# Project-Arda/bgls

Measured on AMD Instinct MI355X. Metric: aggregate-verify signer-pairs/sec, higher is better.
Workload: dtype u32; 1 GPU; altbn128 VerifyAggregateSignature, one 1048576-signer batch, keys+msgs resident in HBM; curve=altbn128, signers=1048576, signers_per_gpu=1048576, in_flight=8

## Files before the change

### __graft_entry__.py

```python
import os
import subprocess
import sys

ROOT = os.path.dirname(os.path.abspath(__file__))
HIPCC = os.environ.get("HIPCC", "/opt/rocm/bin/hipcc")


def _run(cmd, timeout=1800):
    print("+", " ".join(cmd), flush=True)
    subprocess.run(cmd, check=True, cwd=ROOT, timeout=timeout)


def build(force=False):
    csrc = os.path.join(ROOT, "bgls_amd", "csrc")
    jobs = str(min(8, os.cpu_count() or 1))
    _run(["make", "-s", "-j", jobs, "-C", csrc, "HIPCC=" + HIPCC] + (["-B"] if force else []))
    _run(["make", "-s", "-j", jobs, "-C", csrc, "HIPCC=" + HIPCC, "LEGACY=1"] + (["-B"] if force else []))
    omk = os.path.join(ROOT, "oracle", "c", "Makefile")
    if os.path.exists(omk):
        _run(["make", "-s", "-C", os.path.join(ROOT, "oracle", "c")])
    bh_path = os.path.join(ROOT, "tests", "harness", "build_harness.py")
    if os.path.exists(bh_path):
        import importlib.util
        spec = importlib.util.spec_from_file_location("build_harness", bh_path)
        bh = importlib.util.module_from_spec(spec)
        spec.loader.exec_module(bh)
        print("+ host harness (test-only, five parts in parallel)", flush=True)
        bh.build(force=force)
    dh_path = os.path.join(ROOT, "tests", "harness", "build_device_harness.py")
    if os.path.exists(dh_path):
        import importlib.util
        spec = importlib.util.spec_from_file_location("build_device_harness", dh_path)
        dh = importlib.util.module_from_spec(spec)
        spec.loader.exec_module(dh)
        print("+ device harness (test-only, gfx950)", flush=True)
        dh.build(force=force)
    sys.path.insert(0, ROOT)
    import bgls_amd
    from bgls_amd import _lib
    _lib.load()


def smoke():
    sys.path.insert(0, ROOT)
    import ctypes, random
    from bgls_amd import Altbn128, Bls12, bgls, _lib
    from oracle import coracle
    rc = _lib.load().bgls_init(0)
    if rc != 0:
        raise RuntimeError("bgls_init failed: %d %s" % (rc, _lib.last_error()))
    for curve in (Altbn128, Bls12):
        cid = curve.id
        n = 4
        sks = [0x1234567 + 977 * i for i in range(n)]
        msgs = [bytes([i]) * (17 + i) for i in range(n)]
        keys = [curve.GetG2().Mul(sk) for sk in sks]
        sigs = [bgls.Sign(curve, sk, m) for sk, m in zip(sks, msgs)]
        agg = bgls.AggregateSignatures(sigs)
        g2 = curve.GetG2().raw
        okeys = [coracle.scale_point(cid, 2, g2, sk) for sk in sks]
        osigs = [coracle.scale_point(cid, 1, coracle.hash_to_g1(cid, m), sk) for sk, m in zip(sks, msgs)]
        oagg = coracle.aggregate_points(cid, 1, b"".join(osigs), n)
        assert [k.raw for k in keys] == okeys, "public keys differ from oracle"
        assert agg.raw == oagg, "aggregate signature differs from oracle"
        got = bgls.VerifyAggregateSignature(curve, agg, keys, msgs)
        want = coracle.verify_aggregate(cid, oagg, b"".join(okeys), msgs, False, threads=4)
        assert got is True and want == 1, (curve.Name(), got, want)
        bad = bgls.VerifyAggregateSignature(curve, agg, keys, msgs[:-1] + [b"tampered"])
        assert bad is False, "tampered message accepted"
        lib, fp = _lib.load(), curve.fp_bytes
        rnd = random.Random(7)
        n = 150
        sks = [rnd.randrange(1, curve.GetG1Order()) for _ in range(n)]
        kb = (ctypes.c_uint8 * (32 * n)).from_buffer_copy(b"".join(s.to_bytes(32, "big") for s in sks))
        kbuf = (ctypes.c_uint8 * (n * 4 * fp))()
        assert lib.bgls_scale_generator(cid, 2, kb, n, kbuf) == 0
        ms = [rnd.randbytes(32) for _ in range(n)]
        blob = (ctypes.c_uint8 * (32 * n)).from_buffer_copy(b"".join(ms))
        off = (ctypes.c_uint64 * (n + 1))(*range(0, 32 * (n + 1), 32))
        sg = (ctypes.c_uint8 * (n * 2 * fp))()
        assert lib.bgls_sign_batch(cid, kb, blob, off, n, sg) == 0
        ag = (ctypes.c_uint8 * (2 * fp))()
        assert lib.bgls_aggregate_points(cid, 1, sg, n, ag) == 0
        assert lib.bgls_verify_aggregate(cid, ag, kbuf, blob, off, n, 0) == 1
        assert coracle.verify_aggregate(cid, bytes(ag), bytes(kbuf), ms, False, threads=8) == 1, "oracle disagrees on the 150-signer instance"
        blob[32 * 77 + 5] ^= 4
        assert lib.bgls_verify_aggregate(cid, ag, kbuf, blob, off, n, 0) == 0, "tampered 150-signer instance accepted"
        print("smoke ok:", curve.Name())


if __name__ == "__main__":
    build()
    if len(sys.argv) > 1 and sys.argv[1] == "smoke":
        smoke()
```

### bgls_amd/csrc/miller_x.hpp

```cpp
#pragma once
#include <type_traits>
#include "dev_common.hpp"
#include "coop.hpp"
#include "rx_pair.hpp"

namespace bgls {

template <class C>
struct MxForm { typedef C type; };
#ifndef MX_BN_W28
template <>
struct MxForm<BN254> { typedef BN254W type; };
#endif

template <class C, int NP = 60>
struct MX {
  static_assert(NP == 60 || NP == 64, "pairings per block");
  static constexpr int NL = C::RX_NL;
  static constexpr bool PACKED = (C::RX_NL % 4) != 0 && C::CURVE_ID == 1;
  static constexpr int HS = PACKED ? NL : ((NL + 3) & ~3);
  static constexpr int ES = 2 * HS;
  static constexpr int NLINES = NP == 64 ? 7 : 6;
  static constexpr int FOLD_UNROLL = (!rx_lazy<C> && NLINES % 3 == 0) ? 3 : 1;
  static constexpr int KS = PACKED ? 2 * ES : ES;
  static constexpr int WS = PACKED ? 368 : 176;
  static constexpr int GROUP_DW = PACKED ? (NP == 64 ? 940 : 844) : (NP == 64 ? 828 : 764);
  static constexpr int THREADS = 192;
  static __device__ __forceinline__ int acc_off(int k, int wrap) { return k * KS + wrap * WS; }
  static __device__ __forceinline__ int line_off(int e) {
    if constexpr (PACKED) return e < 12 ? 28 + 56 * e + (e >= 6 ? 32 : 0) : (e == 12 ? 336 : 704 + 28 * (e - 13));
    else return 320 + ES * e;
  }
  static_assert(!PACKED || (ES == 28 && 704 + 28 * (3 * NLINES - 13) <= GROUP_DW), "BLS12-381 line slots");
  static_assert(PACKED || 320 + ES * 3 * NLINES <= GROUP_DW, "alt-bn128 line slots");
  static constexpr int PQ = 10 * GROUP_DW;
#ifndef MX_P_LDS_LIMIT
#define MX_P_LDS_LIMIT 40960
#endif
  static constexpr bool P_IN_LDS = (10 * GROUP_DW + NP * 2 * HS) * 4 <= MX_P_LDS_LIMIT;
  static constexpr int SEQ_DW = 10 * GROUP_DW + (P_IN_LDS ? NP * 2 * HS : 0);
#ifdef MX_EXP_FLAGS
  static constexpr int BLOCK_BYTES = (SEQ_DW + 16) * 4;
#else
  static constexpr int BLOCK_BYTES = (10 * GROUP_DW + (P_IN_LDS ? NP * 2 * HS : 0)) * 4;
#endif
  static constexpr int NPARK_Q = C::CURVE_ID == 0 ? 6 : 2;
  static constexpr int NPARK = NPARK_Q + (P_IN_LDS ? 0 : 2);
  static constexpr int PS = (NL + 3) & ~3;
  static constexpr size_t park_bytes(size_t nblocks) { return nblocks * 128 * NPARK * PS * 4; }
};

__device__ __forceinline__ uint4 mx_ld16(int dw) {
  extern __shared__ u32 lds[];
  typedef u32 v4u __attribute__((ext_vector_type(4)));
  const v4u v = *reinterpret_cast<const v4u*>(__builtin_assume_aligned(lds + dw, 16));
  return make_uint4(v.x, v.y, v.z, v.w);
}
template <class C, bool PACKED>
__device__ __forceinline__ Ux<C> mx_ld_half(int off, bool second) {
  constexpr int N = C::RX_NL;
  Ux<C> r;
  if constexpr (!PACKED) {
    (void)second;
#pragma unroll
    for (int k = 0; k < (N + 3) / 4; ++k) {
      const uint4 v = mx_ld16(off + 4 * k);
      r.v[4 * k] = v.x;
      if (4 * k + 1 < N) r.v[4 * k + 1] = v.y;
      if (4 * k + 2 < N) r.v[4 * k + 2] = v.z;
      if (4 * k + 3 < N) r.v[4 * k + 3] = v.w;
    }
  } else {
    static_assert(!PACKED || N % 4 == 2, "packed halves: NL = 2 mod 4");
    if (!second) {
#pragma unroll
      for (int k = 0; k < (N + 2) / 4; ++k) {
        const uint4 v = mx_ld16(off + 4 * k);
        r.v[4 * k] = v.x; r.v[4 * k + 1] = v.y;
        if (4 * k + 2 < N) { r.v[4 * k + 2] = v.z; r.v[4 * k + 3] = v.w; }
      }
    } else {
      const uint4 v0 = mx_ld16(off - 2);
      r.v[0] = v0.z; r.v[1] = v0.w;
#pragma unroll
      for (int k = 1; k < (N + 2) / 4; ++k) {
        const uint4 v = mx_ld16(off - 2 + 4 * k);
        r.v[4 * k - 2] = v.x; r.v[4 * k - 1] = v.y; r.v[4 * k] = v.z; r.v[4 * k + 1] = v.w;
      }
    }
  }
  return r;
}
template <class C, bool PACKED>
__device__ __forceinline__ void mx_st_half(int off, bool second, const Ux<C>& a) {
  extern __shared__ u32 lds[];
  constexpr int N = C::RX_NL;
  if (!PACKED || !second) {
    uint4* p = reinterpret_cast<uint4*>(lds + off);
#pragma unroll
    for (int k = 0; k < N / 4; ++k) p[k] = make_uint4(a.v[4 * k], a.v[4 * k + 1], a.v[4 * k + 2], a.v[4 * k + 3]);
    if constexpr (N % 4 == 2) *reinterpret_cast<uint2*>(lds + off + (N & ~3)) = make_uint2(a.v[N - 2], a.v[N - 1]);
    if constexpr (N % 4 == 1) lds[off + N - 1] = a.v[N - 1];
    static_assert(N % 4 != 3, "tail store");
  } else {
    *reinterpret_cast<uint2*>(lds + off) = make_uint2(a.v[0], a.v[1]);
    uint4* p = reinterpret_cast<uint4*>(lds + off + 2);
#pragma unroll
    for (int k = 0; k < N / 4; ++k) p[k] = make_uint4(a.v[4 * k + 2], a.v[4 * k + 3], a.v[4 * k + 4], a.v[4 * k + 5]);
  }
}

template <class C, class K, bool XI3 = false>
__device__ __forceinline__ void mxk_publish(int gb, int j, const Ux2<C>& v, bool live) {
  if (live) {
    mx_st_half<C, K::PACKED>(gb + K::acc_off(j, 0), false, v.c0);
    mx_st_half<C, K::PACKED>(gb + K::acc_off(j, 0) + K::HS, true, v.c1);
    const Ux2<C> x = ux_mulxi<C>(v);
    if (!XI3 || j >= 3) {
      mx_st_half<C, K::PACKED>(gb + K::acc_off(j, 1), false, x.c0);
      mx_st_half<C, K::PACKED>(gb + K::acc_off(j, 1) + K::HS, true, x.c1);
    }
  }
  wave_sync();
}
template <class C, int NP>
__device__ __forceinline__ void mx_publish(int gb, int j, const Ux2<C>& v, bool live) { mxk_publish<C, MX<C, NP>>(gb, j, v, live); }
template <class C, int NP>
__device__ __forceinline__ Ux2<C> mx_fold(int gb, int m, int j) {
  typedef MX<C, NP> K;
  auto sh = [](int t) { return C::TWIST_D ? t + (t == 2 ? 1 : 0) : t + (t >= 1 ? 1 : 0); };
#ifdef MX_EXP_Q
  if constexpr (C::RX_NL <= 10)
    return ux_dot_k2q<C, 3>(
      [&](int t, int h) { return mx_ld_half<C, K::PACKED>(gb + K::line_off(3 * m + t) + h * K::HS, h != 0); },
      [&](int t, int h) {
        int k = j - sh(t);
        const int wrap = k < 0 ? 1 : 0;
        k += 6 * wrap;
        return mx_ld_half<C, K::PACKED>(gb + K::acc_off(k, wrap) + h * K::HS, h != 0);
      });
  else
#endif
  return ux_dot_k2p<C, 3, (C::RX_NL <= 10)>(
      [&](int t, int h) { return mx_ld_half<C, K::PACKED>(gb + K::line_off(3 * m + t) + h * K::HS, h != 0); },
      [&](int t, int h) {
        int k = j - sh(t);
        const int wrap = k < 0 ? 1 : 0;
        k += 6 * wrap;
        return mx_ld_half<C, K::PACKED>(gb + K::acc_off(k, wrap) + h * K::HS, h != 0);
      });
}
template <class C, class K>
__device__ __forceinline__ Ux2<C> mxk_sqr(int gb, int j) {
  const unsigned row = COOP_SQ_TAB[j];
  return ux_sqr_dot<C>(
      [&](int t) {
        const unsigned e = (row >> (8 * t)) & 0xFFu;
        return (e & 7u) == 7u ? 0 : (((e >> 7) & 1u) ? 2 : 1);
      },
      [&](int t, int h) {
        const unsigned e = (row >> (8 * t)) & 0xFFu;
        const int i = (e & 7u) == 7u ? 0 : (int)(e & 7u);
        return mx_ld_half<C, K::PACKED>(gb + K::acc_off(i, 0) + h * K::HS, h != 0);
      },
      [&](int t, int h) {
        const unsigned e = (row >> (8 * t)) & 0xFFu;
        const bool unused = (e & 7u) == 7u;
        return mx_ld_half<C, K::PACKED>(gb + K::acc_off(unused ? 0 : (int)((e >> 3) & 7u), unused ? 0 : (int)((e >> 6) & 1u)) + h * K::HS, h != 0);
      });
}
template <class C, int NP>
__device__ __forceinline__ Ux2<C> mx_sqr(int gb, int j) { return mxk_sqr<C, MX<C, NP>>(gb, j); }

__device__ __forceinline__ void mx_sq_split(unsigned row, unsigned& pa, unsigned& pb) {
  unsigned d[3] = {0xffu, 0xffu, 0xffu}, p[2] = {0xffu, 0xffu};
  int nd = 0, np = 0;
#pragma unroll
  for (int t = 0; t < 4; ++t) {
    const unsigned e = (row >> (8 * t)) & 0xFFu;
    if ((e & 7u) == 7u) continue;
    if (e & 0x80u) {
      if (nd == 0) d[0] = e; else if (nd == 1) d[1] = e; else d[2] = e;
      ++nd;
    } else {
      if (np == 0) p[0] = e; else p[1] = e;
      ++np;
    }
  }
  if (nd == 3) {
    pa = d[0] | (d[1] << 8) | (1u << 16);
    pb = d[2] | (0xffu << 8);
  } else {
    pa = d[0] | (p[0] << 8);
    pb = d[1] | (p[1] << 8);
  }
}
template <class C, class K>
__device__ __forceinline__ Ux2<C> mxk_sqr3(int gb, unsigned pa, unsigned pb) {
  const bool twice = (pa >> 16) & 1u;
  auto fetch = [&](unsigned sl, int t, int side, int h) __attribute__((always_inline)) {
    const unsigned e = (sl >> (8 * t)) & 0xFFu;
    const bool unused = (e & 7u) == 7u;
    const int i = unused ? 0 : (int)(e & 7u), k = unused ? 0 : (int)((e >> 3) & 7u), wrap = unused ? 0 : (int)((e >> 6) & 1u);
    Ux<C> a = mx_ld_half<C, K::PACKED>(gb + (side == 0 ? K::acc_off(i, 0) : K::acc_off(k, wrap)) + h * K::HS, h != 0);
    if (side == 0) {
      const u32 keep = unused ? 0u : 0xFFFFFFFFu;
#pragma unroll
      for (int q = 0; q < C::RX_NL; ++q) a.v[q] &= keep;
    }
    return a;
  };
  return ux_sqr_dot3<C>([&](int t, int side, int h) { return fetch(pa, t, side, h); }, [&](int t, int side, int h) { return fetch(pb, t, side, h); },
                        [&](int t) { return t == 0 && !twice; }, [&](int t) { return t == 0; }, twice);
}

template <class C, int NP>
__device__ __forceinline__ Ux2<C> mx_sqr3(int gb, unsigned pa, unsigned pb) { return mxk_sqr3<C, MX<C, NP>>(gb, pa, pb); }

template <class C>
struct MxPark {
  static constexpr int NL = C::RX_NL;
  static constexpr int HS = MX<C>::PS;
  static __device__ __forceinline__ void st_raw(u32* lane_base, int slot, const u32 (&v)[NL]) {
    uint4* p = reinterpret_cast<uint4*>(lane_base + slot * HS);
#pragma unroll
    for (int k = 0; k < NL / 4; ++k) p[k] = make_uint4(v[4 * k], v[4 * k + 1], v[4 * k + 2], v[4 * k + 3]);
    if constexpr (NL % 4 == 2) *reinterpret_cast<uint2*>(lane_base + slot * HS + (NL & ~3)) = make_uint2(v[NL - 2], v[NL - 1]);
    if constexpr (NL % 4 == 1) lane_base[slot * HS + NL - 1] = v[NL - 1];
  }
  static __device__ __forceinline__ void ld_raw(const u32* lane_base, int slot, u32 (&v)[NL]) {
    const uint4* p = reinterpret_cast<const uint4*>(lane_base + slot * HS);
#pragma unroll
    for (int k = 0; k < NL / 4; ++k) {
// ... 97 lines not shown
    role = w == cw ? 2 : (w > cw ? w - 1 : w);
  } else {
    const int rot = rmode == 2 ? (int)(blockIdx.x % 3u) : 0;
    role = w + rot;
    if (role >= 3) role -= 3;
  }
#ifdef MX_EXP_FLAGS
  if (threadIdx.x < 4) lds_roles[K::SEQ_DW + threadIdx.x] = 0u;
  __syncthreads();
#endif
  u32* srec = nullptr;
  int sstep = 0;
  if constexpr (DBG == 4) {
    if (rec_dbg != nullptr && blockIdx.x % MX_STAMP_EVERY == 0) {
      srec = rec_dbg + ((size_t)(blockIdx.x / MX_STAMP_EVERY) * 3 + w) * MX_STAMP_DW;
      if (lane == 0) {
        const unsigned long long t = __builtin_amdgcn_s_memrealtime();
        srec[0] = __builtin_amdgcn_s_getreg((31 << 11) | 4);
        srec[1] = __builtin_amdgcn_s_getreg((31 << 11) | 20);
        srec[2] = (u32)t; srec[3] = (u32)(t >> 32);
        srec[6] = (u32)role;
        srec[7] = (u32)__builtin_readcyclecounter();
      }
    }
  }
  if (role < 2) {
    if (rot_mode & 8) __builtin_amdgcn_s_setprio(3);
    const int q = lane >> 1;
    const bool odd = lane & 1;
    const bool owner = q < PPW;
    const int pi = role * PPW + (owner ? q : 0);
    const size_t idx = (size_t)blockIdx.x * NP + pi;
    const int tg = pi < 60 ? pi / 6 : pi - 60, m = pi < 60 ? pi % 6 : 6;
    u32* const mypark = park + ((size_t)blockIdx.x * 128 + (role * 64 + lane)) * (K::NPARK * K::PS);
    constexpr int P_NYP = K::NPARK_Q, P_XP = K::NPARK_Q + 1;
    bool valid = owner && idx < n;
    PointX<C> T;
    {
      constexpr int NB = C::FP_BYTES;
      const uint8_t* kb = g2s + (valid ? idx : 0) * 4 * NB;
      const Fp<C> xw = fp_from_be<C>(kb + (odd ? 0 : NB)), yw = fp_from_be<C>(kb + (odd ? 2 * NB : 3 * NB));
      const bool canon_own = !fp_geq_p<C>(xw) && !fp_geq_p<C>(yw);
      const bool zero_own = fp_is_zero<C>(xw) && fp_is_zero<C>(yw);
      const bool canon = canon_own && pair_swap1(canon_own ? 1 : 0) != 0;
      const bool qinf = zero_own && pair_swap1(zero_own ? 1 : 0) != 0;
      Sx<C, SX_T> xq = sx_from_plain<C>(xw), yq = sx_from_plain<C>(yw);
      {
        const Sx<C, SX_T> b2 = sx_const<C>(odd ? C::RX_B2_IM : C::RX_B2_RE);
        const auto d = sx_sub<C>(pair_sqr<C>(yq, odd), sx_add<C>(pair_mul<C>(pair_sqr<C>(xq, odd), xq, odd), b2));
        const bool on_own = sx_is_zero_mod_p<C>(d);
        const bool on_curve = on_own && pair_swap1(on_own ? 1 : 0) != 0;
        if (valid && !(canon && (qinf || on_curve))) atomicOr(flags, FLAG_ENC);
      }
      Aff<F1<C>> P = g1s[valid ? idx : 0];
      valid = valid && !P.inf && !qinf;
      if (!valid) {
        xq = ux_to_sx<C>(to_ux<C>(fp_load<C>(C::G2 + (odd ? C::L : 0))));
        yq = ux_to_sx<C>(to_ux<C>(fp_load<C>(C::G2 + 2 * C::L + (odd ? C::L : 0))));
        P.x = fp_load<C>(C::G1X);
        P.y = fp_load<C>(C::G1Y);
      }
      MxPark<C>::st(mypark, 0, xq);
      MxPark<C>::st(mypark, 1, yq);
      if constexpr (C::CURVE_ID == 0) {
        const Sx<C, SX_T> cx = sx_select<C>(odd, sx_neg<C>(xq), xq), cy = sx_select<C>(odd, sx_neg<C>(yq), yq);
        constexpr int N2 = 2 * C::RX_NL;
        MxPark<C>::st(mypark, 2, pair_mul_const<C>(cx, C::RX_GAMMA + 0 * N2, C::RX_GAMMA + 0 * N2 + C::RX_NL, odd));
        MxPark<C>::st(mypark, 3, pair_mul_const<C>(cy, C::RX_GAMMA + 1 * N2, C::RX_GAMMA + 1 * N2 + C::RX_NL, odd));
        MxPark<C>::st(mypark, 4, pair_mul_const<C>(xq, C::RX_GAMMA + 2 * N2, C::RX_GAMMA + 2 * N2 + C::RX_NL, odd));
        MxPark<C>::st(mypark, 5, sx_norm<C>(sx_neg<C>(pair_mul_const<C>(yq, C::RX_GAMMA + 3 * N2, C::RX_GAMMA + 3 * N2 + C::RX_NL, odd))));
      }
      if constexpr (K::P_IN_LDS) {
        if (owner) mx_st_half<C, K::PACKED>(K::PQ + (2 * pi + (odd ? 1 : 0)) * K::HS, odd, odd ? to_ux<C>(P.x) : to_ux<C>(fp_neg<C>(P.y)));
        wave_sync();
      } else {
        MxPark<C>::st(mypark, P_NYP, ux_to_sx<C>(to_ux<C>(fp_neg<C>(P.y))));
        MxPark<C>::st(mypark, P_XP, ux_to_sx<C>(to_ux<C>(P.x)));
      }
      T.X = xq;
      T.Y = yq;
      T.Z = sx_select<C>(odd, ux_to_sx<C>(ux_zero<C>()), sx_const<C>(C::RX_ONE));
    }
    const int rl_base = tg * K::GROUP_DW + (odd ? K::HS : 0);
    Ux<C> e[3];
    auto emit = [&](int which, const auto& v) __attribute__((always_inline)) {
      const int entry = which == 1 ? 1 : ((which == 0) == C::TWIST_D ? 0 : 2);
      if constexpr (rx_lazy<C>) e[entry] = sx_to_ux<C>(v);
      else if constexpr (std::is_same<std::decay_t<decltype(v)>, Sx<C, SX_T>>::value) e[entry] = sx_to_ux_p<C>(v);
      else e[entry] = sx_to_ux_k<1, C>(v);
    };
    int pstep = 0;
    auto hand_over = [&]() __attribute__((always_inline)) {
      if (DBG == 2 || __builtin_amdgcn_ballot_w64(owner && !valid) != 0) {
        if (DBG == 2 || !valid) {
          e[0] = odd ? ux_zero<C>() : ux_load<C>(C::RX_ONE);
          e[1] = ux_zero<C>();
          e[2] = ux_zero<C>();
        }
      }
      mx_stamp<DBG>(srec, 16 + 4 * sstep);
#ifdef MX_EXP_FLAGS
      mx_seq_wait(K::SEQ_DW, 2 * pstep + 2 - (MX_EXP_FLAGS));
#else
      __syncthreads();
#endif
      mx_stamp<DBG>(srec, 16 + 4 * sstep + 1);
      if (owner) {
        mx_st_half<C, K::PACKED>(rl_base + K::line_off(3 * m), odd, e[0]);
        mx_st_half<C, K::PACKED>(rl_base + K::line_off(3 * m + 1), odd, e[1]);
        mx_st_half<C, K::PACKED>(rl_base + K::line_off(3 * m + 2), odd, e[2]);
      }
      mx_stamp<DBG>(srec, 16 + 4 * sstep + 2);
#ifdef MX_EXP_FLAGS
      ++pstep;
      mx_seq_st(K::SEQ_DW + 1 + role, (u32)pstep);
#else
      __syncthreads();
#endif
      mx_stamp<DBG>(srec, 16 + 4 * sstep + 3);
      if constexpr (DBG == 4) ++sstep;
    };
    struct Env {
      const u32* pk;
      int xs, ys;
      bool neg_y;
      int pq;
      __device__ __forceinline__ Sx<C, SX_T> nyP() const {
        if constexpr (K::P_IN_LDS) return ux_to_sx<C>(mx_ld_half<C, K::PACKED>(pq, false));
        else return MxPark<C>::ld(MxPark<C>::launder(pk), K::NPARK_Q);
      }
      __device__ __forceinline__ Sx<C, SX_T> xP() const {
        if constexpr (K::P_IN_LDS) return ux_to_sx<C>(mx_ld_half<C, K::PACKED>(pq + K::HS, true));
        else return MxPark<C>::ld(MxPark<C>::launder(pk), K::NPARK_Q + 1);
      }
      __device__ __forceinline__ Sx<C, SX_T> xq() const { return MxPark<C>::ld(MxPark<C>::launder(pk), xs); }
      __device__ __forceinline__ Sx<C, SX_T> yq() const {
        const Sx<C, SX_T> y = MxPark<C>::ld(MxPark<C>::launder(pk), ys);
        return sx_select<C>(neg_y, sx_neg<C>(y), y);
      }
    };
#pragma unroll 1
    for (int i = 1; i < C::LOOP_LEN; ++i) {
      if constexpr (DBG != 2) dbl_step_x<C>(T, Env{mypark, 0, 1, false, K::PQ + 2 * pi * K::HS}, odd, emit);
      hand_over();
      const int d = C::LOOP_NAF[i];
      if (d != 0) {
        if constexpr (DBG != 2) add_step_x<C>(T, Env{mypark, 0, 1, d < 0, K::PQ + 2 * pi * K::HS}, odd, emit);
        hand_over();
      }
    }
    if constexpr (C::CURVE_ID == 0) {
#pragma unroll 1
      for (int s = 0; s < 2; ++s) {
        if constexpr (DBG != 2) add_step_x<C>(T, Env{mypark, 2 + 2 * s, 3 + 2 * s, false, K::PQ + 2 * pi * K::HS}, odd, emit);
        hand_over();
      }
    }
    if constexpr (DBG == 0) {
      const bool z_own = sx_is_zero_mod_p<C>(T.Z);
      const bool z_zero = z_own && pair_swap1(z_own ? 1 : 0) != 0;
      if (valid && z_zero && !odd) atomicOr(flags, FLAG_DEGENERATE);
    }
  } else {
    if (rot_mode & 4) __builtin_amdgcn_s_setprio(3);
#ifdef MX_PRIO_EXP
    if (((rot_mode >> 5) & 3) == 1) __builtin_amdgcn_s_setprio(1);
    if (((rot_mode >> 5) & 3) == 2) __builtin_amdgcn_s_setprio(2);
#endif
    const bool live = lane < 60;
    const int cl = live ? lane : lane - 12;
    const int g = cl % 10;
    const int j = cl / 10;
    const int gb = g * K::GROUP_DW;
    Ux2<C> fj;
    {
      const Ux<C> one = ux_load<C>(C::RX_ONE);
#pragma unroll
      for (int k = 0; k < NL; ++k) { fj.c0.v[k] = j == 0 ? one.v[k] : 0u; fj.c1.v[k] = 0u; }
    }
    if constexpr (NP == 64) {
      if (live && g >= 4 && j < 3) {
        const Ux<C> one = ux_load<C>(C::RX_ONE), zero = ux_zero<C>();
        mx_st_half<C, K::PACKED>(gb + K::line_off(18 + j), false, j == 0 ? one : zero);
        mx_st_half<C, K::PACKED>(gb + K::line_off(18 + j) + K::HS, true, zero);
      }
    }
    mx_publish<C, NP>(gb, j, fj, live);
    unsigned sq_d = 0, sq_p = 0;
    int cstep = 0;
    (void)cstep;
    if constexpr (!rx_lazy<C>) mx_sq_split(COOP_SQ_TAB[j], sq_d, sq_p);
    auto fold_all = [&]() __attribute__((always_inline)) {
      if constexpr (DBG == 1) {
#ifdef MX_EXP_FLAGS
        mx_seq_st(K::SEQ_DW, (u32)(2 * cstep + 2));
        ++cstep;
#endif
        return;
      }
#pragma unroll K::FOLD_UNROLL
      for (int m = 0; m < K::NLINES; ++m) {
        fj = mx_fold<C, NP>(gb, m, j);
#ifdef MX_EXP_FLAGS
        if (m == 2) mx_seq_st(K::SEQ_DW, (u32)(2 * cstep + 1));
        if (m == K::NLINES - 1) mx_seq_st(K::SEQ_DW, (u32)(2 * cstep + 2));
#endif
        mx_publish<C, NP>(gb, j, fj, live);
      }
#ifdef MX_EXP_FLAGS
      ++cstep;
#endif
    };
#ifdef MX_EXP_FLAGS
    auto lines_ready = [&]() __attribute__((always_inline)) {
      mx_seq_wait(K::SEQ_DW + 1, cstep + 1);
      mx_seq_wait(K::SEQ_DW + 2, cstep + 1);
    };
#endif
#pragma unroll 1
    for (int i = 1; i < C::LOOP_LEN; ++i) {
#ifndef MX_SQR_LATE
      if (DBG != 1 && i > 1) {
        if constexpr (rx_lazy<C>) fj = mx_sqr<C, NP>(gb, j);
        else fj = mx_sqr3<C, NP>(gb, sq_d, sq_p);
        mx_publish<C, NP>(gb, j, fj, live);
      }
#endif
      mx_stamp<DBG>(srec, 16 + 4 * sstep);
#ifdef MX_EXP_FLAGS
      lines_ready();
#else
      __syncthreads();
#endif
      mx_stamp<DBG>(srec, 16 + 4 * sstep + 1);
#ifdef MX_SQR_LATE
      if (DBG != 1 && i > 1) {
        if constexpr (rx_lazy<C>) fj = mx_sqr<C, NP>(gb, j);
        else fj = mx_sqr3<C, NP>(gb, sq_d, sq_p);
        mx_publish<C, NP>(gb, j, fj, live);
      }
#endif
      mx_stamp<DBG>(srec, 16 + 4 * sstep + 2);
#ifndef MX_EXP_FLAGS
      __syncthreads();
#endif
      mx_stamp<DBG>(srec, 16 + 4 * sstep + 3);
      if constexpr (DBG == 4) ++sstep;
      fold_all();
      if (C::LOOP_NAF[i] != 0) {
        mx_stamp<DBG>(srec, 16 + 4 * sstep);
#ifdef MX_EXP_FLAGS
        lines_ready();
#else
        __syncthreads();
#endif
        mx_stamp<DBG>(srec, 16 + 4 * sstep + 1);
        mx_stamp<DBG>(srec, 16 + 4 * sstep + 2);
#ifndef MX_EXP_FLAGS
        __syncthreads();
#endif
        mx_stamp<DBG>(srec, 16 + 4 * sstep + 3);
        if constexpr (DBG == 4) ++sstep;
        fold_all();
      }
    }
    if constexpr (C::CURVE_ID == 0) {
#pragma unroll 1
      for (int s = 0; s < 2; ++s) {
        mx_stamp<DBG>(srec, 16 + 4 * sstep);
#ifdef MX_EXP_FLAGS
        lines_ready();
#else
        __syncthreads();
#endif
        mx_stamp<DBG>(srec, 16 + 4 * sstep + 1);
        mx_stamp<DBG>(srec, 16 + 4 * sstep + 2);
#ifndef MX_EXP_FLAGS
        __syncthreads();
#endif
        mx_stamp<DBG>(srec, 16 + 4 * sstep + 3);
        if constexpr (DBG == 4) ++sstep;
        fold_all();
      }
    }
    if (live) {
      if constexpr (!rx_lazy<C>) fj = ux_quasi<C, 2, 1>(fj);
      Fp2<C> r = {from_ux_inl<C>(fj.c0), from_ux_inl<C>(fj.c1)};
      if constexpr (C::CURVE_ID != 0) {
        if (j & 1) r = f2_neg<C>(r);
      }
      out[((size_t)blockIdx.x * 10 + g) * 6 + j] = r;
    }
  }
  if constexpr (DBG == 3) {
    if (lane == 0) {
      u32* rec = rec_dbg + ((size_t)blockIdx.x * 3 + w) * 8;
      const unsigned long long t = __builtin_amdgcn_s_memrealtime();
      rec[4] = (u32)t; rec[5] = (u32)(t >> 32);
      rec[6] = (u32)role;
    }
  }
  if constexpr (DBG == 4) {
    if (srec != nullptr && lane == 0) {
      const unsigned long long t = __builtin_amdgcn_s_memrealtime();
      srec[4] = (u32)t; srec[5] = (u32)(t >> 32);
      srec[8] = (u32)__builtin_readcyclecounter();
      srec[9] = (u32)sstep;
    }
  }
}

}
```

### bgls_amd/csrc/rx.hpp

```cpp
#pragma once
#include "tower.hpp"

namespace bgls {

typedef int32_t i32;
typedef int64_t i64;
constexpr u32 RX_MASK = (1u << 28) - 1;
template <class C>
constexpr bool rx_lazy = 2 * C::RX_W + 8 <= 64;
template <class C>
constexpr bool rx_fits(long long budget) { return (long long)C::RX_NL * (budget + 256) + 64 < (1ll << (71 - 2 * C::RX_W)); }

#if !defined(__HIP_DEVICE_COMPILE__) && defined(BGLS_RX_CHECK)
extern int g_rx_overflow;
#define RX_HOST_CHECK 1
#else
#define RX_HOST_CHECK 0
#endif

BGLS_HD void rx_macu(u64& c, u32 a, u32 b) {
#if defined(__HIP_DEVICE_COMPILE__)
  asm volatile("v_mad_u64_u32 %0, vcc, %1, %2, %0" : "+v"(c) : "v"(a), "v"(b) : "vcc");
#elif RX_HOST_CHECK
  u64 r;
// ... 165 lines not shown
    r.v[i] = t & C::RX_MASK;
    c = t >> C::RX_W;
  }
  r.v[C::RX_NL - 1] = a.v[C::RX_NL - 1] + c;
  return r;
}

template <class C>
BGLS_HD Ux2<C> ux_mulxi(const Ux2<C>& a) {
  Ux2<C> r;
  if constexpr (rx_lazy<C>) {
#pragma unroll
    for (int i = 0; i < C::RX_NL; ++i) {
      r.c0.v[i] = (u32)C::XI_RE * a.c0.v[i] + (C::RX_FAT[i] - a.c1.v[i]);
      r.c1.v[i] = (u32)C::XI_RE * a.c1.v[i] + a.c0.v[i];
    }
    r.c0 = ux_norm<C>(r.c0);
    r.c1 = ux_norm<C>(r.c1);
  } else {
    constexpr int T = C::RX_NL - 1;
    constexpr float QI = 1.0f / (float)(C::RX_P[T] + 1u);
#if RX_HOST_CHECK
    for (int i = 0; i < T; ++i)
      if (a.c0.v[i] > C::RX_MASK || a.c1.v[i] > C::RX_MASK) g_rx_overflow = 1;
    if (a.c0.v[T] > 3u * C::RX_P[T] + 3u || a.c1.v[T] > 3u * C::RX_P[T] + 3u) g_rx_overflow = 1;
#endif
    const i32 s0 = (i32)((u32)C::XI_RE * a.c0.v[T]) - (i32)a.c1.v[T] + 4 * (i32)C::RX_P[T];
    const i32 s1 = (i32)((u32)C::XI_RE * a.c1.v[T] + a.c0.v[T]);
    auto quot = [&](i32 s) {
      i32 q = (i32)((float)s * QI) - 2;
      q = q < 0 ? 0 : q;
      return (u32)(32 - (q > 31 ? 31 : q));
    };
    const u32 k0 = quot(s0), k1 = quot(s1);
    u64 c0 = 0, c1 = 0;
#pragma unroll
    for (int i = 0; i < T; ++i) {
      const u64 t0 = (u64)(u32)C::XI_RE * a.c0.v[i] + (u64)k0 * C::RX_P[i] + (u64)((u32)C::RX_XIG0[i] - a.c1.v[i]) + c0;
      const u64 t1 = (u64)(u32)C::XI_RE * a.c1.v[i] + (u64)k1 * C::RX_P[i] + (u64)((u32)C::RX_XIG1[i] + a.c0.v[i]) + c1;
      r.c0.v[i] = (u32)t0 & C::RX_MASK;
      r.c1.v[i] = (u32)t1 & C::RX_MASK;
      c0 = t0 >> C::RX_W;
      c1 = t1 >> C::RX_W;
    }
    r.c0.v[T] = (u32)((i32)((u32)C::XI_RE * a.c0.v[T] + k0 * C::RX_P[T]) + (i32)C::RX_XIG0[T] - (i32)a.c1.v[T] + (i32)c0);
    r.c1.v[T] = (u32)((i32)((u32)C::XI_RE * a.c1.v[T] + k1 * C::RX_P[T] + a.c0.v[T]) + (i32)C::RX_XIG1[T] + (i32)c1);
#if RX_HOST_CHECK
    if ((i32)r.c0.v[T] < 0 || (i32)r.c1.v[T] < 0 || r.c0.v[T] > 3u * C::RX_P[T] + 3u || r.c1.v[T] > 3u * C::RX_P[T] + 3u) g_rx_overflow = 1;
#endif
  }
  return r;
}

template <class C, int KHI, int KLO>
BGLS_HD Ux<C> ux_quasi(const Ux<C>& a) {
  constexpr int N = C::RX_NL;
  static_assert(KLO >= 1 && KHI <= 6 && KHI - KLO <= 3, "ladder levels");
  i32 t[N];
#pragma unroll
  for (int i = 0; i < N; ++i) t[i] = (i32)a.v[i];
#pragma unroll
  for (int k = KHI; k >= KLO; --k) {
    const u32* L = C::RX_LAD + (k - 1) * N;
    const i32 hit = t[N - 1] >= (i32)L[N - 1] + 5 ? -1 : 0;
#pragma unroll
    for (int i = 0; i < N; ++i) t[i] -= (i32)L[i] & hit;
  }
  Ux<C> r;
  i32 c = 0;
#pragma unroll
  for (int i = 0; i < N - 1; ++i) {
    const i32 s = t[i] + c;
    r.v[i] = (u32)(s & (i32)C::RX_MASK);
    c = s >> C::RX_W;
  }
  r.v[N - 1] = (u32)(t[N - 1] + c);
  return r;
}
template <class C, int KHI, int KLO>
BGLS_HD Ux2<C> ux_quasi(const Ux2<C>& a) {
  return {ux_quasi<C, KHI, KLO>(a.c0), ux_quasi<C, KHI, KLO>(a.c1)};
}

template <class C, int NT, bool PF = false, class LA, class LB>
BGLS_HD Ux2<C> ux_dot_k2p(LA&& lda, LB&& ldb) {
  constexpr int N = C::RX_NL;
  static_assert(NT >= 1 && NT <= 3, "column budget");
  u64 d[2 * N], e[2 * N];
  if constexpr (PF) {
    Ux<C> a0 = lda(0, 0), b0 = ldb(0, 0);
    {
      const Ux<C> a1 = lda(0, 1), b1 = ldb(0, 1);
      ux_acc_new<C>(d, a0, b0);
      if (NT > 1) { a0 = lda(1, 0); b0 = ldb(1, 0); }
      ux_acc_new<C>(e, a1, b1);
    }
#pragma unroll 1
    for (int t = 1; t < NT; ++t) {
      const Ux<C> a1 = lda(t, 1), b1 = ldb(t, 1);
      ux_acc<C>(d, a0, b0);
      if (t + 1 < NT) { a0 = lda(t + 1, 0); b0 = ldb(t + 1, 0); }
      ux_acc<C>(e, a1, b1);
    }
  } else {
    {
      const Ux<C> a0 = lda(0, 0), b0 = ldb(0, 0);
      ux_acc_new<C>(d, a0, b0);
    }
    {
      const Ux<C> a1 = lda(0, 1), b1 = ldb(0, 1);
      ux_acc_new<C>(e, a1, b1);
    }
#pragma unroll
    for (int t = 1; t < NT; ++t) {
      {
        const Ux<C> a0 = lda(t, 0), b0 = ldb(t, 0);
        ux_acc<C>(d, a0, b0);
      }
      {
        const Ux<C> a1 = lda(t, 1), b1 = ldb(t, 1);
        ux_acc<C>(e, a1, b1);
      }
    }
  }
  Ux2<C> r;
#pragma unroll
  for (int k = 0; k < 2 * N; ++k) {
    const u64 dk = d[k], ek = e[k];
    e[k] = dk + C::RX_BIAS_D3[k] - ek;
    d[k] = dk + ek;
  }
  r.c0 = ux_redc<C>(e);
#if RX_HOST_CHECK
  u64 chk[2 * N];
  for (int k = 0; k < 2 * N; ++k) chk[k] = 0;
#endif
#pragma unroll
  for (int t = 0; t < NT; ++t) {
    i32 sa[N], sb[N];
    {
      const Ux<C> a0 = lda(t, 0), a1 = lda(t, 1);
#pragma unroll
      for (int q = 0; q < N; ++q) sa[q] = (i32)a1.v[q] - (i32)a0.v[q];
    }
    {
      const Ux<C> b0 = ldb(t, 0), b1 = ldb(t, 1);
#pragma unroll
      for (int q = 0; q < N; ++q) sb[q] = (i32)b0.v[q] - (i32)b1.v[q];
    }
#if RX_HOST_CHECK
    ux_acc<C>(chk, lda(t, 0), ldb(t, 1));
    ux_acc<C>(chk, lda(t, 1), ldb(t, 0));
#endif
#pragma unroll
    for (int i = 0; i < N; ++i) rx_rows_wrap<N>(d + i, sa[i], sb);
  }
#if RX_HOST_CHECK
  for (int k = 0; k < 2 * N; ++k)
    if (chk[k] != d[k]) g_rx_overflow = 1;
#endif
  r.c1 = ux_redc<C>(d);
  return r;
}

template <class C, int NT, class LA, class LB>
BGLS_HD Ux2<C> ux_dot_k2q(LA&& lda, LB&& ldb) {
// ... 539 lines not shown
```

### bgls_amd/csrc/rx_pair.hpp

```cpp
#pragma once
#include "rx.hpp"

#if defined(__HIPCC__)
#define RX_DEV __device__ __forceinline__
#else
#define RX_DEV inline __attribute__((always_inline))
int rx_host_pair_swap(int v);
#endif

namespace bgls {

RX_DEV i32 pair_swap1(i32 v) {
#if defined(__HIPCC__)
  return __builtin_amdgcn_update_dpp(0, v, 0xB1 , 0xF, 0xF, true);
#else
  return rx_host_pair_swap(v);
#endif
}
RX_DEV i32 pair_even1(i32 v, bool odd) {
#if defined(__HIPCC__)
  (void)odd;
  return __builtin_amdgcn_update_dpp(0, v, 0xA0 , 0xF, 0xF, true);
#else
  const i32 o = rx_host_pair_swap(v);
  return odd ? o : v;
#endif
}
RX_DEV i32 pair_odd1(i32 v, bool odd) {
#if defined(__HIPCC__)
  (void)odd;
  return __builtin_amdgcn_update_dpp(0, v, 0xF5 , 0xF, 0xF, true);
#else
  const i32 o = rx_host_pair_swap(v);
  return odd ? v : o;
#endif
}
template <class C, int LA>
RX_DEV Sx<C, LA> pair_swap_neg_even(const Sx<C, LA>& a, bool odd) {
  const i32 sgn = odd ? 0 : -1;
  Sx<C, LA> r;
#pragma unroll
  for (int i = 0; i < C::RX_NL; ++i) r.v[i] = (pair_swap1(a.v[i]) ^ sgn) - sgn;
  return r;
}

template <class C, int LA, int LB>
RX_DEV Sx<C, SX_T> pair_mul(const Sx<C, LA>& a, const Sx<C, LB>& b, bool odd) {
  const Sx<C, LA> pa = pair_swap_neg_even<C>(a, odd);
  const i32* const cols[2] = {a.v, pa.v};
  return sx_montr<C, 2, 2 * LA * LB>(cols, [&](int k, int i) { return k == 0 ? pair_even1(b.v[i], odd) : pair_odd1(b.v[i], odd); });
}
template <class C, int LA>
RX_DEV Sx<C, SX_T> pair_mul_const(const Sx<C, LA>& a, const u32* k_re, const u32* k_im, bool odd) {
  const Sx<C, LA> pa = pair_swap_neg_even<C>(a, odd);
  const i32* const cols[2] = {a.v, pa.v};
  return sx_montr<C, 2, 2 * LA * SX_T>(cols, [&](int k, int i) { return (i32)(k == 0 ? k_re[i] : k_im[i]); });
}
template <class C, int LA>
RX_DEV Sx<C, SX_T> pair_sqr(const Sx<C, LA>& a, bool odd) {
  static_assert(rx_lazy<C> || LA <= SX_F, "29-bit form: squares of (nearly) non-negative limbs only");
  constexpr int BUDGET = rx_lazy<C> ? 4 * LA * LA : 2 * LA * (LA + 1);
  Sx<C, 2 * LA> u;
#pragma unroll
  for (int i = 0; i < C::RX_NL; ++i) u.v[i] = a.v[i] + pair_odd1(a.v[i], odd);
  const i32 even = odd ? 0 : -1;
  const i32* const cols[1] = {u.v};
  return sx_montr<C, 1, BUDGET>(cols, [&](int, int i) { return pair_even1(a.v[i], odd) - (pair_odd1(a.v[i], odd) & even); });
}
template <class C, int LA, int LS>
RX_DEV Sx<C, SX_T> pair_muls(const Sx<C, LA>& a, const Sx<C, LS>& s) {
  const i32* const cols[1] = {s.v};
  return sx_montr<C, 1, LA * LS>(cols, [&](int, int i) { return a.v[i]; });
}
template <class C, int LA, int LB, int LC, int LD>
RX_DEV Sx<C, SX_T> pair_mulsub(const Sx<C, LA>& a, const Sx<C, LB>& b, const Sx<C, LC>& c, const Sx<C, LD>& d, bool odd) {
  static_assert(rx_fits<C>(2 * LA * LB + 2 * LC * LD), "four products per reduction: 28-bit forms (the 29-bit form reduces the two products apart)");
  const Sx<C, LA> pa = pair_swap_neg_even<C>(a, odd);
  const Sx<C, LC> pc = pair_swap_neg_even<C>(c, odd);
  const i32* const cols[4] = {a.v, pa.v, c.v, pc.v};
  return sx_montr<C, 4, 2 * LA * LB + 2 * LC * LD>(cols, [&](int k, int i) {
    return k == 0 ? pair_even1(b.v[i], odd) : (k == 1 ? pair_odd1(b.v[i], odd) : (k == 2 ? -pair_even1(d.v[i], odd) : -pair_odd1(d.v[i], odd)));
  });
}
template <class C, int LG, int LE, int LF>
RX_DEV Sx<C, SX_T> pair_sqrsub(const Sx<C, LG>& g, const Sx<C, LE>& e, const Sx<C, LF>& f, bool odd) {
  static_assert(rx_fits<C>(4 * LG * LG + 2 * LE * LF), "three products per reduction: 28-bit forms");
  Sx<C, 2 * LG> u;
#pragma unroll
  for (int i = 0; i < C::RX_NL; ++i) u.v[i] = g.v[i] + pair_odd1(g.v[i], odd);
  const i32 even = odd ? 0 : -1;
  const Sx<C, LE> pe = pair_swap_neg_even<C>(e, odd);
  const i32* const cols[3] = {u.v, e.v, pe.v};
  return sx_montr<C, 3, 4 * LG * LG + 2 * LE * LF>(cols, [&](int k, int i) {
    return k == 0 ? pair_even1(g.v[i], odd) - (pair_odd1(g.v[i], odd) & even) : (k == 1 ? -pair_even1(f.v[i], odd) : -pair_odd1(f.v[i], odd));
  });
}
template <class C, int LG, int LE>
RX_DEV Sx<C, SX_T> pair_sqrsub3(const Sx<C, LG>& g, const Sx<C, LE>& e, bool odd) {
  static_assert(LG <= SX_F && LE <= SX_T, "g: a reduction's output or one carry step behind a sum; e: a reduction's output");
  constexpr int BUDGET = 513 + 6 * LE * LE;
  static_assert(rx_fits<C>(BUDGET), "two squares per reduction: 28-bit forms");
  Sx<C, 2 * LG> u;
  Sx<C, 2 * LE> w;
#pragma unroll
  for (int i = 0; i < C::RX_NL; ++i) {
    u.v[i] = g.v[i] + pair_odd1(g.v[i], odd);
    w.v[i] = e.v[i] + pair_odd1(e.v[i], odd);
  }
  const i32 even = odd ? 0 : -1;
  const i32* const cols[2] = {u.v, w.v};
  return sx_montr<C, 2, BUDGET>(cols, [&](int k, int i) {
    return k == 0 ? pair_even1(g.v[i], odd) - (pair_odd1(g.v[i], odd) & even) : -3 * (pair_even1(e.v[i], odd) - (pair_odd1(e.v[i], odd) & even));
  });
}
template <class C, int LA>
RX_DEV Sx<C, SX_T> pair_mul_3b(const Sx<C, LA>& z, bool odd) {
  if constexpr (C::CURVE_ID == 1) {
    static_assert(C::XI_RE == 1 && !C::TWIST_D, "3 b' = 12 (1 + i): BLS12-381's M-type twist");
    const auto t = sx_normf<C>(sx_add<C>(z, pair_swap_neg_even<C>(z, odd)));
    const auto t12 = sx_mulc<4, C>(sx_normf<C>(sx_mulc<3, C>(t)));
    return sx_quasi_center<C>(t12);
  } else {
    return pair_mul_const<C>(z, C::RX_B2X3_RE, C::RX_B2X3_IM, odd);
  }
}
// ... 55 lines not shown
```

Baseline: 18.72 million signer-pairs/s.

## Add XL Miller-loop form storing xi-multiplied line coefficients in LDS

Adds an XL variant of the cooperative Miller-loop kernel for the 29-bit alt-bn128 form with 60 pairings per block, enabled by default. Line-producing threads now also emit xi-multiplied copies of two line entries, using a new per-half multiply-by-xi with a quotient estimate. The fold step reads these precomputed copies instead of wrapping accumulators. Publish skips the xi multiply except before a squaring. The LDS layout is reworked to 1020 dwords per group so four blocks fit per CU, with the hash points kept in the workspace. The intent is to take xi multiplications off the fold and publish critical path, at the cost of more line stores and LDS footprint.

```diff
diff --git a/__graft_entry__.py b/__graft_entry__.py
--- a/__graft_entry__.py
+++ b/__graft_entry__.py
@@ -27,6 +27,14 @@
         spec.loader.exec_module(bh)
         print("+ host harness (test-only, five parts in parallel)", flush=True)
         bh.build(force=force)
+    xh_path = os.path.join(ROOT, "tests", "harness", "build_harness_xl.py")
+    if os.path.exists(xh_path):
+        import importlib.util
+        spec = importlib.util.spec_from_file_location("build_harness_xl", xh_path)
+        xh = importlib.util.module_from_spec(spec)
+        spec.loader.exec_module(xh)
+        print("+ host harness of the Miller kernel's XL form (test-only)", flush=True)
+        xh.build(force=force)
     dh_path = os.path.join(ROOT, "tests", "harness", "build_device_harness.py")
     if os.path.exists(dh_path):
         import importlib.util
diff --git a/bgls_amd/csrc/miller_x.hpp b/bgls_amd/csrc/miller_x.hpp
--- a/bgls_amd/csrc/miller_x.hpp
+++ b/bgls_amd/csrc/miller_x.hpp
@@ -13,9 +13,18 @@
 struct MxForm<BN254> { typedef BN254W type; };
 #endif
 
-template <class C, int NP = 60>
+template <class C, int NP>
+struct MxXlDefault { static constexpr bool value = false; };
+#ifndef MX_NO_XL
+template <>
+struct MxXlDefault<BN254W, 60> { static constexpr bool value = true; };
+#endif
+
+template <class C, int NP = 60, bool XL_ = MxXlDefault<C, NP>::value>
 struct MX {
   static_assert(NP == 60 || NP == 64, "pairings per block");
+  static constexpr bool XL = XL_;
+  static_assert(!XL || (NP == 60 && !rx_lazy<C> && C::TWIST_D && C::RX_NL <= 12), "XL: the 29-bit form's 60-pairing block, D-type twist");
   static constexpr int NL = C::RX_NL;
   static constexpr bool PACKED = (C::RX_NL % 4) != 0 && C::CURVE_ID == 1;
   static constexpr int HS = PACKED ? NL : ((NL + 3) & ~3);
@@ -23,8 +32,8 @@
   static constexpr int NLINES = NP == 64 ? 7 : 6;
   static constexpr int FOLD_UNROLL = (!rx_lazy<C> && NLINES % 3 == 0) ? 3 : 1;
   static constexpr int KS = PACKED ? 2 * ES : ES;
-  static constexpr int WS = PACKED ? 368 : 176;
-  static constexpr int GROUP_DW = PACKED ? (NP == 64 ? 940 : 844) : (NP == 64 ? 828 : 764);
+  static constexpr int WS = XL ? 112 : (PACKED ? 368 : 176);
+  static constexpr int GROUP_DW = XL ? 1020 : (PACKED ? (NP == 64 ? 940 : 844) : (NP == 64 ? 828 : 764));
   static constexpr int THREADS = 192;
   static __device__ __forceinline__ int acc_off(int k, int wrap) { return k * KS + wrap * WS; }
   static __device__ __forceinline__ int line_off(int e) {
@@ -32,7 +41,11 @@
     else return 320 + ES * e;
   }
   static_assert(!PACKED || (ES == 28 && 704 + 28 * (3 * NLINES - 13) <= GROUP_DW), "BLS12-381 line slots");
-  static_assert(PACKED || 320 + ES * 3 * NLINES <= GROUP_DW, "alt-bn128 line slots");
+  static_assert(PACKED || XL || 320 + ES * 3 * NLINES <= GROUP_DW, "alt-bn128 line slots");
+  static __device__ __forceinline__ int line_off_x(int m, int t, bool xi, bool glo) {
+    return t == 0 ? 256 + ES * m : (t == 1 ? (xi ? 544 + (glo ? 8 : 0) : 400) + ES * m : (xi ? 696 : 840) + ES * m);
+  }
+  static_assert(!XL || (ES == 24 && KS == 24 && WS + 3 * KS >= 6 * KS && WS + 6 * KS <= 256 && 840 + 6 * ES <= GROUP_DW), "XL line slots");
   static constexpr int PQ = 10 * GROUP_DW;
 #ifndef MX_P_LDS_LIMIT
 #define MX_P_LDS_LIMIT 40960
@@ -43,6 +56,7 @@
   static constexpr int BLOCK_BYTES = (SEQ_DW + 16) * 4;
 #else
   static constexpr int BLOCK_BYTES = (10 * GROUP_DW + (P_IN_LDS ? NP * 2 * HS : 0)) * 4;
+  static_assert(!XL || (BLOCK_BYTES <= 40960 && !P_IN_LDS), "XL: four blocks per CU; the hash points' coordinates are parked in the workspace");
 #endif
   static constexpr int NPARK_Q = C::CURVE_ID == 0 ? 6 : 2;
   static constexpr int NPARK = NPARK_Q + (P_IN_LDS ? 0 : 2);
@@ -110,24 +124,41 @@
   }
 }
 
-template <class C, class K, bool XI3 = false>
-__device__ __forceinline__ void mxk_publish(int gb, int j, const Ux2<C>& v, bool live) {
+template <class C, class K, bool XI3 = false, bool XL = false>
+__device__ __forceinline__ void mxk_publish(int gb, int j, const Ux2<C>& v, bool live, bool sq_next = true) {
   if (live) {
     mx_st_half<C, K::PACKED>(gb + K::acc_off(j, 0), false, v.c0);
     mx_st_half<C, K::PACKED>(gb + K::acc_off(j, 0) + K::HS, true, v.c1);
-    const Ux2<C> x = ux_mulxi<C>(v);
-    if (!XI3 || j >= 3) {
-      mx_st_half<C, K::PACKED>(gb + K::acc_off(j, 1), false, x.c0);
-      mx_st_half<C, K::PACKED>(gb + K::acc_off(j, 1) + K::HS, true, x.c1);
+    if constexpr (XL) {
+      if (j >= 3) {
+        Ux2<C> x = v;
+        if (sq_next) x = ux_mulxi<C>(v);
+        mx_st_half<C, K::PACKED>(gb + K::acc_off(j, 1), false, x.c0);
+        mx_st_half<C, K::PACKED>(gb + K::acc_off(j, 1) + K::HS, true, x.c1);
+      }
+    } else {
+      const Ux2<C> x = ux_mulxi<C>(v);
+      if (!XI3 || j >= 3) {
+        mx_st_half<C, K::PACKED>(gb + K::acc_off(j, 1), false, x.c0);
+        mx_st_half<C, K::PACKED>(gb + K::acc_off(j, 1) + K::HS, true, x.c1);
+      }
     }
   }
   wave_sync();
 }
 template <class C, int NP>
-__device__ __forceinline__ void mx_publish(int gb, int j, const Ux2<C>& v, bool live) { mxk_publish<C, MX<C, NP>>(gb, j, v, live); }
+__device__ __forceinline__ void mx_publish(int gb, int j, const Ux2<C>& v, bool live, bool sq_next = false) {
+  mxk_publish<C, MX<C, NP>, false, MX<C, NP>::XL>(gb, j, v, live, sq_next);
+}
 template <class C, int NP>
-__device__ __forceinline__ Ux2<C> mx_fold(int gb, int m, int j) {
+__device__ __forceinline__ Ux2<C> mx_fold(int gb, int m, int j, bool glo = false) {
   typedef MX<C, NP> K;
+  if constexpr (K::XL) {
+    return ux_dot_k2p<C, 3, (C::RX_NL <= 10)>(
+        [&](int t, int h) { return mx_ld_half<C, K::PACKED>(gb + K::line_off_x(m, t, mxl_wraps<C>(j, t), glo) + h * K::HS, h != 0); },
+        [&](int t, int h) { return mx_ld_half<C, K::PACKED>(gb + K::acc_off(mxl_acc_k<C>(j, t), mxl_wraps<C>(j, t) ? 1 : 0) + h * K::HS, h != 0); });
+  } else {
+  (void)glo;
   auto sh = [](int t) { return C::TWIST_D ? t + (t == 2 ? 1 : 0) : t + (t >= 1 ? 1 : 0); };
 #ifdef MX_EXP_Q
   if constexpr (C::RX_NL <= 10)
@@ -149,6 +180,7 @@
         k += 6 * wrap;
         return mx_ld_half<C, K::PACKED>(gb + K::acc_off(k, wrap) + h * K::HS, h != 0);
       });
+  }
 }
 template <class C, class K>
 __device__ __forceinline__ Ux2<C> mxk_sqr(int gb, int j) {
@@ -412,12 +444,15 @@
       T.Z = sx_select<C>(odd, ux_to_sx<C>(ux_zero<C>()), sx_const<C>(C::RX_ONE));
     }
     const int rl_base = tg * K::GROUP_DW + (odd ? K::HS : 0);
-    Ux<C> e[3];
+    Ux<C> e[K::XL ? 5 : 3];
     auto emit = [&](int which, const auto& v) __attribute__((always_inline)) {
       const int entry = which == 1 ? 1 : ((which == 0) == C::TWIST_D ? 0 : 2);
       if constexpr (rx_lazy<C>) e[entry] = sx_to_ux<C>(v);
       else if constexpr (std::is_same<std::decay_t<decltype(v)>, Sx<C, SX_T>>::value) e[entry] = sx_to_ux_p<C>(v);
       else e[entry] = sx_to_ux_k<1, C>(v);
+      if constexpr (K::XL) {
+        if (entry != 0) e[entry + 2] = pair_mulxi_half<C>(e[entry], odd);
+      }
     };
     int pstep = 0;
     auto hand_over = [&]() __attribute__((always_inline)) {
@@ -426,6 +461,7 @@
           e[0] = odd ? ux_zero<C>() : ux_load<C>(C::RX_ONE);
           e[1] = ux_zero<C>();
           e[2] = ux_zero<C>();
+          if constexpr (K::XL) { e[3] = ux_zero<C>(); e[4] = ux_zero<C>(); }
         }
       }
       mx_stamp<DBG>(srec, 16 + 4 * sstep);
@@ -436,9 +472,16 @@
 #endif
       mx_stamp<DBG>(srec, 16 + 4 * sstep + 1);
       if (owner) {
-        mx_st_half<C, K::PACKED>(rl_base + K::line_off(3 * m), odd, e[0]);
-        mx_st_half<C, K::PACKED>(rl_base + K::line_off(3 * m + 1), odd, e[1]);
-        mx_st_half<C, K::PACKED>(rl_base + K::line_off(3 * m + 2), odd, e[2]);
+        if constexpr (K::XL) {
+#pragma unroll
+          for (int t = 0; t < 3; ++t) mx_st_half<C, K::PACKED>(rl_base + K::line_off_x(m, t, false, tg < 6), odd, e[t]);
+          mx_st_half<C, K::PACKED>(rl_base + K::line_off_x(m, 1, true, tg < 6), odd, e[3]);
+          mx_st_half<C, K::PACKED>(rl_base + K::line_off_x(m, 2, true, tg < 6), odd, e[4]);
+        } else {
+          mx_st_half<C, K::PACKED>(rl_base + K::line_off(3 * m), odd, e[0]);
+          mx_st_half<C, K::PACKED>(rl_base + K::line_off(3 * m + 1), odd, e[1]);
+          mx_st_half<C, K::PACKED>(rl_base + K::line_off(3 * m + 2), odd, e[2]);
+        }
       }
       mx_stamp<DBG>(srec, 16 + 4 * sstep + 2);
 #ifdef MX_EXP_FLAGS
@@ -502,6 +545,7 @@
     const int g = cl % 10;
     const int j = cl / 10;
     const int gb = g * K::GROUP_DW;
+    const bool glo = g < 6;
     Ux2<C> fj;
     {
       const Ux<C> one = ux_load<C>(C::RX_ONE);
@@ -520,7 +564,7 @@
     int cstep = 0;
     (void)cstep;
     if constexpr (!rx_lazy<C>) mx_sq_split(COOP_SQ_TAB[j], sq_d, sq_p);
-    auto fold_all = [&]() __attribute__((always_inline)) {
+    auto fold_all = [&](bool sq_next) __attribute__((always_inline)) {
       if constexpr (DBG == 1) {
 #ifdef MX_EXP_FLAGS
         mx_seq_st(K::SEQ_DW, (u32)(2 * cstep + 2));
@@ -530,12 +574,12 @@
       }
 #pragma unroll K::FOLD_UNROLL
       for (int m = 0; m < K::NLINES; ++m) {
-        fj = mx_fold<C, NP>(gb, m, j);
+        fj = mx_fold<C, NP>(gb, m, j, glo);
 #ifdef MX_EXP_FLAGS
         if (m == 2) mx_seq_st(K::SEQ_DW, (u32)(2 * cstep + 1));
         if (m == K::NLINES - 1) mx_seq_st(K::SEQ_DW, (u32)(2 * cstep + 2));
 #endif
-        mx_publish<C, NP>(gb, j, fj, live);
+        mx_publish<C, NP>(gb, j, fj, live, sq_next && m == K::NLINES - 1);
       }
 #ifdef MX_EXP_FLAGS
       ++cstep;
@@ -576,7 +620,7 @@
 #endif
       mx_stamp<DBG>(srec, 16 + 4 * sstep + 3);
       if constexpr (DBG == 4) ++sstep;
-      fold_all();
+      fold_all(C::LOOP_NAF[i] == 0 && i + 1 < C::LOOP_LEN);
       if (C::LOOP_NAF[i] != 0) {
         mx_stamp<DBG>(srec, 16 + 4 * sstep);
 #ifdef MX_EXP_FLAGS
@@ -591,7 +635,7 @@
 #endif
         mx_stamp<DBG>(srec, 16 + 4 * sstep + 3);
         if constexpr (DBG == 4) ++sstep;
-        fold_all();
+        fold_all(i + 1 < C::LOOP_LEN);
       }
     }
     if constexpr (C::CURVE_ID == 0) {
@@ -610,7 +654,7 @@
 #endif
         mx_stamp<DBG>(srec, 16 + 4 * sstep + 3);
         if constexpr (DBG == 4) ++sstep;
-        fold_all();
+        fold_all(false);
       }
     }
     if (live) {
diff --git a/bgls_amd/csrc/rx.hpp b/bgls_amd/csrc/rx.hpp
--- a/bgls_amd/csrc/rx.hpp
+++ b/bgls_amd/csrc/rx.hpp
@@ -271,6 +271,16 @@
   return {ux_quasi<C, KHI, KLO>(a.c0), ux_quasi<C, KHI, KLO>(a.c1)};
 }
 
+template <class C>
+BGLS_HD int mxl_sh(int t) { return C::TWIST_D ? t + (t == 2 ? 1 : 0) : t + (t >= 1 ? 1 : 0); }
+template <class C>
+BGLS_HD bool mxl_wraps(int j, int t) { return j < mxl_sh<C>(t); }
+template <class C>
+BGLS_HD int mxl_acc_k(int j, int t) {
+  const int k = j - mxl_sh<C>(t);
+  return k < 0 ? k + 6 : k;
+}
+
 template <class C, int NT, bool PF = false, class LA, class LB>
 BGLS_HD Ux2<C> ux_dot_k2p(LA&& lda, LB&& ldb) {
   constexpr int N = C::RX_NL;
diff --git a/bgls_amd/csrc/rx_pair.hpp b/bgls_amd/csrc/rx_pair.hpp
--- a/bgls_amd/csrc/rx_pair.hpp
+++ b/bgls_amd/csrc/rx_pair.hpp
@@ -41,6 +41,39 @@
   Sx<C, LA> r;
 #pragma unroll
   for (int i = 0; i < C::RX_NL; ++i) r.v[i] = (pair_swap1(a.v[i]) ^ sgn) - sgn;
+  return r;
+}
+
+template <class C>
+RX_DEV Ux<C> pair_mulxi_half(const Ux<C>& a, bool odd) {
+  static_assert(!rx_lazy<C>, "the lazy forms multiply by xi without a quotient (ux_mulxi)");
+  constexpr int T = C::RX_NL - 1;
+  constexpr float QI = 1.0f / (float)(C::RX_P[T] + 1u);
+  Ux<C> b;
+#pragma unroll
+  for (int i = 0; i <= T; ++i) b.v[i] = (u32)pair_swap1((i32)a.v[i]);
+#if RX_HOST_CHECK
+  for (int i = 0; i < T; ++i)
+    if (a.v[i] > C::RX_MASK) g_rx_overflow = 1;
+  if (3u * a.v[T] > 10u * C::RX_P[T]) g_rx_overflow = 1;
+#endif
+  const i32 s = (i32)((u32)C::XI_RE * a.v[T]) + (odd ? (i32)b.v[T] : 4 * (i32)C::RX_P[T] - (i32)b.v[T]);
+  i32 q = (i32)((float)s * QI) - 2;
+  q = q < 0 ? 0 : q;
+  const u32 k = (u32)(32 - (q > 31 ? 31 : q));
+  Ux<C> r;
+  u64 c = 0;
+#pragma unroll
+  for (int i = 0; i < T; ++i) {
+    const u32 g = odd ? (u32)C::RX_XIG1[i] + b.v[i] : (u32)C::RX_XIG0[i] - b.v[i];
+    const u64 t = (u64)(u32)C::XI_RE * a.v[i] + (u64)k * C::RX_P[i] + (u64)g + c;
+    r.v[i] = (u32)t & C::RX_MASK;
+    c = t >> C::RX_W;
+  }
+  r.v[T] = (u32)((i32)((u32)C::XI_RE * a.v[T] + k * C::RX_P[T]) + (odd ? (i32)C::RX_XIG1[T] + (i32)b.v[T] : (i32)C::RX_XIG0[T] - (i32)b.v[T]) + (i32)c);
+#if RX_HOST_CHECK
+  if ((i32)r.v[T] < 0 || r.v[T] > 3u * C::RX_P[T] + 3u) g_rx_overflow = 1;
+#endif
   return r;
 }
 
```

Result: faster. 18.98 million signer-pairs/s (median of 6 runs) (+1.4%).
